# rubengooj/pl-slam

Hardware: AMD Instinct MI355X
Metric: stereo pairs/sec (1500 ORB + 200 LBD BF-match) (higher is better)
Workload: dtype fp4; 1 GPU; C2: synthetic 752x480 stereo stream, 1500 ORB + 200 LBD per image, ORB+LBD L<->R and prev<->curr, mutual + ratio (StVO::match), then StereoFrame's gates over the L<->R tables (config_kitti.yaml:25-...; mutual=True, distinct_batches_in_rotation=3, stereo_gates=True, kernel=k_scan_sym_mfma_i, mfma_form=0

## Files before the change

### plslam_amd/csrc/hamming.hip

```cpp
#include "mfma_h_common.hpp"
#include "stereo_gates_dev.hpp"

namespace plslam {

typedef const __attribute__((address_space(4))) uint32_t* sptr_t;
typedef uint32_t u32x4 __attribute__((ext_vector_type(4), aligned(4)));

__device__ __forceinline__ uint32_t bcnt0(uint32_t x)
{
    uint32_t r;
    asm("v_bcnt_u32_b32 %0, %1, 0" : "=v"(r) : "v"(x));
    return r;
}
__device__ __forceinline__ uint32_t med3_u32(uint32_t a, uint32_t b, uint32_t c)
{
    uint32_t r;
    asm("v_med3_u32 %0, %1, %2, %3" : "=v"(r) : "v"(a), "v"(b), "v"(c));
    return r;
}
__device__ __forceinline__ uint32_t make_key_s(uint32_t d, uint32_t j_uniform)
{
    uint32_t r;
    asm("v_lshl_or_b32 %0, %1, 23, %2" : "=v"(r) : "v"(d), "s"(j_uniform));
    return r;
// ... 134 lines not shown
    for (int k = 0; k < WPQ_QUERIES_PER_WAVE; ++k) {
        uint32_t k0 = b[k][0], k1 = b[k][1];
#pragma unroll
        for (int m = 32; m >= 1; m >>= 1)
            merge2(k0, k1, (uint32_t)__shfl_xor((int)k0, m), (uint32_t)__shfl_xor((int)k1, m));
        if (lane == 0 && q0 + k < nq) g_(reinterpret_cast<gvec2_t*>(sc.keys))[q0 + k] = gvec2_t{k0, k1};
    }
}

constexpr int SYM_TILE_ROW_U16 = 72;
constexpr int SYM_TILE_U16 = 64 * SYM_TILE_ROW_U16;

typedef uint16_t u16x2 __attribute__((ext_vector_type(2)));

constexpr uint32_t SYM_INVALID_BIAS = 512;
__device__ __forceinline__ uint32_t pk_keys(uint32_t w, uint32_t ipair_uniform)
{
    uint32_t r;
    asm("v_lshl_or_b32 %0, %1, 6, %2" : "=v"(r) : "v"(w), "s"(ipair_uniform));
    return r;
}
__device__ __forceinline__ uint32_t key16_to_32(uint32_t c, uint32_t i_base)
{
    return c >= 0x8000u ? KEY_NONE : (((c >> 6) << KEY_IDX_BITS) | (i_base + (c & 63u)));
}

__device__ __forceinline__ void sym_column_reduce(const uint16_t* __restrict__ col, uint32_t& b0,
                                                  uint32_t& b1)
{
    const uint4* cp = reinterpret_cast<const uint4*>(col);
    b0 = 0xFFFFFFFFu;
    b1 = 0xFFFFFFFFu;
#pragma unroll
    for (int v = 0; v < 8; ++v) {
        const uint4 w4 = cp[v];
        const uint32_t w[4] = {w4.x, w4.y, w4.z, w4.w};
#pragma unroll
        for (int u = 0; u < 4; ++u) {
            const int i_lo = 8 * v + 2 * u;
            const uint32_t key = pk_keys(w[u], (uint32_t)(((i_lo + 1) << 16) | i_lo));
            pk_push2(b0, b1, key);
        }
    }
}

__global__ void __launch_bounds__(256)
k_scan_symmetric(const SymDesc* __restrict__ syms, const BlockDesc* __restrict__ blocks,
                 int32_t* __restrict__ zero, int nzero)
{
    __shared__ __attribute__((aligned(16))) uint16_t lds[4 * SYM_TILE_U16];

    if (blockIdx.x == 0)
        for (int i = threadIdx.x; i < nzero; i += 256) g_(zero)[i] = 0;

    const int wg = xcd_remap_(blockIdx.x, gridDim.x);
    const BlockDesc bd = blocks[wg];
    if (bd.item < 0) return;
    const SymDesc sd = syms[bd.item];
    const int n1 = sd.n1, n2 = sd.n2;
    const int lane = threadIdx.x & 63;
    const int wave = __builtin_amdgcn_readfirstlane((int)(threadIdx.x >> 6));
    const int i0 = bd.row0 + 64 * wave;
    if (i0 >= n1) return;
    const int iblk = i0 >> 6;
    const int row = i0 + lane;
    const uint32_t bias = row < n1 ? 0u : SYM_INVALID_BIAS;
    const int rrow = row < n1 ? row : n1 - 1;

    uint32_t q[8];
    {
        const auto qp = g_(reinterpret_cast<const u32x4*>(sd.a + (size_t)rrow * 32));
        const u32x4 a = qp[0], b = qp[1];
        q[0] = a.x; q[1] = a.y; q[2] = a.z; q[3] = a.w;
        q[4] = b.x; q[5] = b.y; q[6] = b.z; q[7] = b.w;
    }
    uint16_t* tile = lds + wave * SYM_TILE_U16;
    uint16_t* wr = tile + lane;
    const uint16_t* col = tile + lane * SYM_TILE_ROW_U16;
    const auto part = g_(reinterpret_cast<gvec2_t*>(sd.part21)) + (size_t)iblk * n2;
    sptr_t tp = (sptr_t)(uintptr_t)sd.b;

    uint32_t rb0 = KEY_NONE, rb1 = KEY_NONE;
    for (int j0 = 0; j0 < n2; j0 += 64) {
        const int jc = n2 - j0 < 64 ? n2 - j0 : 64;
        int jj = 0;
        for (; jj + 4 <= jc; jj += 4) {
            sptr_t t = tp + (size_t)(j0 + jj) * 8;
            const uint32_t d0 = PLSLAM_DIST8B(q, t, bias);
            const uint32_t d1 = PLSLAM_DIST8B(q, t + 8, bias);
            const uint32_t d2 = PLSLAM_DIST8B(q, t + 16, bias);
            const uint32_t d3 = PLSLAM_DIST8B(q, t + 24, bias);
            wr[(jj + 0) * SYM_TILE_ROW_U16] = (uint16_t)d0;
            wr[(jj + 1) * SYM_TILE_ROW_U16] = (uint16_t)d1;
            wr[(jj + 2) * SYM_TILE_ROW_U16] = (uint16_t)d2;
            wr[(jj + 3) * SYM_TILE_ROW_U16] = (uint16_t)d3;
            best2_push(rb0, rb1, make_key_s(d0, (uint32_t)(j0 + jj)));
            best2_push(rb0, rb1, make_key_s(d1, (uint32_t)(j0 + jj + 1)));
            best2_push(rb0, rb1, make_key_s(d2, (uint32_t)(j0 + jj + 2)));
            best2_push(rb0, rb1, make_key_s(d3, (uint32_t)(j0 + jj + 3)));
        }
        for (; jj < jc; ++jj) {
            sptr_t t = tp + (size_t)(j0 + jj) * 8;
            const uint32_t d = PLSLAM_DIST8B(q, t, bias);
            wr[jj * SYM_TILE_ROW_U16] = (uint16_t)d;
            best2_push(rb0, rb1, make_key_s(d, (uint32_t)(j0 + jj)));
        }
        __builtin_amdgcn_fence(__ATOMIC_RELEASE, "wavefront");
        __builtin_amdgcn_wave_barrier();
        __builtin_amdgcn_fence(__ATOMIC_ACQUIRE, "wavefront");
        uint32_t c0p, c1p;
        sym_column_reduce(col, c0p, c1p);
        {
            const uint32_t e0 = c0p & 0xFFFFu, o0 = c0p >> 16, e1 = c1p & 0xFFFFu, o1 = c1p >> 16;
            const uint32_t m0 = umin_(e0, o0);
            const uint32_t m1 = umin_(umax_(e0, o0), umin_(e1, o1));
            if (lane < jc)
                part[j0 + lane] = gvec2_t{key16_to_32(m0, (uint32_t)i0), key16_to_32(m1, (uint32_t)i0)};
        }
        __builtin_amdgcn_fence(__ATOMIC_RELEASE, "wavefront");
        __builtin_amdgcn_wave_barrier();
        __builtin_amdgcn_fence(__ATOMIC_ACQUIRE, "wavefront");
    }
    if (row < n1) g_(reinterpret_cast<gvec2_t*>(sd.keys12))[row] = gvec2_t{rb0, rb1};
}

constexpr int SYM4_SUBTILE_U16 = 16 * SYM_TILE_ROW_U16;

__global__ void __launch_bounds__(64)
k_scan_symmetric_r4(const SymDesc* __restrict__ syms, const BlockDesc* __restrict__ blocks,
                    int32_t* __restrict__ zero, int nzero)
{
    __shared__ __attribute__((aligned(16))) uint16_t tile[4 * SYM4_SUBTILE_U16];

    if (blockIdx.x == 0)
        for (int i = threadIdx.x; i < nzero; i += 64) g_(zero)[i] = 0;

    const int wg = xcd_remap_(blockIdx.x, gridDim.x);
    const BlockDesc bd = blocks[wg];
    if (bd.item < 0) return;
    const SymDesc sd = syms[bd.item];
    const int n1 = sd.n1, n2 = sd.n2;
    const int lane = threadIdx.x;
    const int i0 = bd.row0;
    const int iblk = i0 >> 8;

    uint32_t q0[8], c1[8], c2[8], c3[8];
    uint32_t bias[4];
    {
        uint32_t qr[4][8];
#pragma unroll
        for (int r = 0; r < 4; ++r) {
            const int row = i0 + 64 * r + lane;
            bias[r] = row < n1 ? 0u : SYM_INVALID_BIAS;
            const int rrow = row < n1 ? row : n1 - 1;
            const auto qp = g_(reinterpret_cast<const u32x4*>(sd.a + (size_t)rrow * 32));
            const u32x4 a = qp[0], b = qp[1];
            qr[r][0] = a.x; qr[r][1] = a.y; qr[r][2] = a.z; qr[r][3] = a.w;
            qr[r][4] = b.x; qr[r][5] = b.y; qr[r][6] = b.z; qr[r][7] = b.w;
        }
#pragma unroll
        for (int k = 0; k < 8; ++k) {
            q0[k] = qr[0][k];
            c1[k] = qr[0][k] ^ qr[1][k];
            c2[k] = qr[0][k] ^ qr[2][k];
            c3[k] = qr[0][k] ^ qr[3][k];
        }
    }
    uint16_t* wr = tile + lane;
    const uint16_t* col = tile + (lane >> 4) * SYM4_SUBTILE_U16 + (lane & 15) * SYM_TILE_ROW_U16;
    const uint32_t col_i_base = (uint32_t)(i0 + 64 * (lane >> 4));
    const auto part = g_(reinterpret_cast<gvec2_t*>(sd.part21)) + (size_t)iblk * n2;
    sptr_t tp = (sptr_t)(uintptr_t)sd.b;

    uint32_t rb[4][2];
#pragma unroll
    for (int r = 0; r < 4; ++r) rb[r][0] = rb[r][1] = KEY_NONE;

#define PLSLAM_SYM4_ROW(T, JJ)                                                                    \
    {                                                                                             \
        uint32_t x[8];                                                                            \
        _Pragma("unroll") for (int k = 0; k < 8; ++k) x[k] = q0[k] ^ (T)[k];                      \
        const uint32_t e0 = bcnt_acc_(x[7], bcnt_acc_(x[6], bcnt_acc_(x[5], bcnt_acc_(x[4],       \
                            bcnt_acc_(x[3], bcnt_acc_(x[2], bcnt_acc_(x[1], bcnt_acc_(x[0], bias[0])))))))); \
        const uint32_t e1 = bcnt_acc_(x[7] ^ c1[7], bcnt_acc_(x[6] ^ c1[6], bcnt_acc_(x[5] ^ c1[5], \
                            bcnt_acc_(x[4] ^ c1[4], bcnt_acc_(x[3] ^ c1[3], bcnt_acc_(x[2] ^ c1[2], \
                            bcnt_acc_(x[1] ^ c1[1], bcnt_acc_(x[0] ^ c1[0], bias[1]))))))));      \
        const uint32_t e2 = bcnt_acc_(x[7] ^ c2[7], bcnt_acc_(x[6] ^ c2[6], bcnt_acc_(x[5] ^ c2[5], \
                            bcnt_acc_(x[4] ^ c2[4], bcnt_acc_(x[3] ^ c2[3], bcnt_acc_(x[2] ^ c2[2], \
                            bcnt_acc_(x[1] ^ c2[1], bcnt_acc_(x[0] ^ c2[0], bias[2]))))))));      \
        const uint32_t e3 = bcnt_acc_(x[7] ^ c3[7], bcnt_acc_(x[6] ^ c3[6], bcnt_acc_(x[5] ^ c3[5], \
                            bcnt_acc_(x[4] ^ c3[4], bcnt_acc_(x[3] ^ c3[3], bcnt_acc_(x[2] ^ c3[2], \
                            bcnt_acc_(x[1] ^ c3[1], bcnt_acc_(x[0] ^ c3[0], bias[3]))))))));      \
        wr[0 * SYM4_SUBTILE_U16 + (JJ) * SYM_TILE_ROW_U16] = (uint16_t)e0;                        \
        wr[1 * SYM4_SUBTILE_U16 + (JJ) * SYM_TILE_ROW_U16] = (uint16_t)e1;                        \
        wr[2 * SYM4_SUBTILE_U16 + (JJ) * SYM_TILE_ROW_U16] = (uint16_t)e2;                        \
        wr[3 * SYM4_SUBTILE_U16 + (JJ) * SYM_TILE_ROW_U16] = (uint16_t)e3;                        \
        const uint32_t jkey = (uint32_t)(j0 + (JJ));                                              \
        best2_push(rb[0][0], rb[0][1], make_key_s(e0, jkey));                                     \
        best2_push(rb[1][0], rb[1][1], make_key_s(e1, jkey));                                     \
        best2_push(rb[2][0], rb[2][1], make_key_s(e2, jkey));                                     \
        best2_push(rb[3][0], rb[3][1], make_key_s(e3, jkey));                                     \
    }

    for (int j0 = 0; j0 < n2; j0 += 16) {
        const int jc = n2 - j0 < 16 ? n2 - j0 : 16;
        int jj = 0;
        for (; jj + 4 <= jc; jj += 4) {
            sptr_t t = tp + (size_t)(j0 + jj) * 8;
            PLSLAM_SYM4_ROW(t, jj + 0)
            PLSLAM_SYM4_ROW(t + 8, jj + 1)
            PLSLAM_SYM4_ROW(t + 16, jj + 2)
            PLSLAM_SYM4_ROW(t + 24, jj + 3)
        }
        for (; jj < jc; ++jj) {
            sptr_t t = tp + (size_t)(j0 + jj) * 8;
            PLSLAM_SYM4_ROW(t, jj)
        }
        __builtin_amdgcn_fence(__ATOMIC_RELEASE, "wavefront");
        __builtin_amdgcn_wave_barrier();
        __builtin_amdgcn_fence(__ATOMIC_ACQUIRE, "wavefront");
        uint32_t c0p, c1p;
        sym_column_reduce(col, c0p, c1p);
        const uint32_t ev0 = c0p & 0xFFFFu, od0 = c0p >> 16, ev1 = c1p & 0xFFFFu, od1 = c1p >> 16;
        uint32_t k0 = key16_to_32(umin_(ev0, od0), col_i_base);
        uint32_t k1 = key16_to_32(umin_(umax_(ev0, od0), umin_(ev1, od1)), col_i_base);
        merge2(k0, k1, (uint32_t)__shfl_xor((int)k0, 16), (uint32_t)__shfl_xor((int)k1, 16));
        merge2(k0, k1, (uint32_t)__shfl_xor((int)k0, 32), (uint32_t)__shfl_xor((int)k1, 32));
        if (lane < jc) part[j0 + lane] = gvec2_t{k0, k1};
        __builtin_amdgcn_fence(__ATOMIC_RELEASE, "wavefront");
        __builtin_amdgcn_wave_barrier();
        __builtin_amdgcn_fence(__ATOMIC_ACQUIRE, "wavefront");
    }
#undef PLSLAM_SYM4_ROW
#pragma unroll
    for (int r = 0; r < 4; ++r) {
        const int row = i0 + 64 * r + lane;
        if (row < n1) g_(reinterpret_cast<gvec2_t*>(sd.keys12))[row] = gvec2_t{rb[r][0], rb[r][1]};
    }
}

__global__ void __launch_bounds__(256)
k_merge_partials(const SymDesc* __restrict__ syms, const BlockDesc* __restrict__ blocks)
{
    const BlockDesc bd = blocks[blockIdx.x];
    const SymDesc sd = syms[bd.item];
    const int j = bd.row0 + (int)threadIdx.x;
    if (j >= sd.n2) return;
    const auto part = g_(reinterpret_cast<const gvec2_t*>(sd.part21));
    uint32_t b0 = KEY_NONE, b1 = KEY_NONE;
    for (int ib = 0; ib < sd.n_iblk; ++ib) {
        const gvec2_t p = part[(size_t)ib * sd.n2 + j];
        merge2(b0, b1, p.x, p.y);
    }
    g_(reinterpret_cast<gvec2_t*>(sd.keys21))[j] = gvec2_t{b0, b1};
}

__device__ __forceinline__ int ratio_pick(uint32_t k0, uint32_t k1, float nnr)
{
    if (k1 == KEY_NONE) return -1;
    const float d0 = (float)(k0 >> KEY_IDX_BITS);
    const float d1n = __fmul_rn((float)(k1 >> KEY_IDX_BITS), nnr);
    return d0 < d1n ? (int)(k0 & KEY_IDX_MASK) : -1;
}

template <class FetchKb>
__device__ __forceinline__ void finalize_row(const ProblemDesc& p, const int i1, const plslam_stereo_gate_problem* __restrict__ gates,
                                             FetchKb fetch_kb, const gvec2_t* pre = nullptr)
{
    int m = -1;
    bool accepted = false, cleared = false;
    uint2 k = make_uint2(KEY_NONE, KEY_NONE);
    uint2 kb = make_uint2(KEY_NONE, KEY_NONE);
    bool check = false;
    if (i1 < p.n1) {
        if (p.nsplit > 1) {
            const auto tmp = g_(reinterpret_cast<const gvec2_t*>(p.split_tmp));
            uint32_t b0 = KEY_NONE, b1 = KEY_NONE;
            for (int s = 0; s < p.nsplit; ++s) {
                const gvec2_t q = tmp[(size_t)s * p.n1 + i1];
                const uint32_t off = (uint32_t)(s * p.cstep);
                merge2(b0, b1, q.x == KEY_NONE ? KEY_NONE : q.x + off, q.y == KEY_NONE ? KEY_NONE : q.y + off);
            }
            k = make_uint2(b0, b1);
            g_(reinterpret_cast<gvec2_t*>(p.keys12_out))[i1] = gvec2_t{k.x, k.y};
        } else if (pre) {
            k = make_uint2(pre->x, pre->y);
        } else {
            const gvec2_t kv = __builtin_nontemporal_load(g_(reinterpret_cast<const gvec2_t*>(p.keys12)) + i1);
            k = make_uint2(kv.x, kv.y);
        }
        m = ratio_pick(k.x, k.y, p.nnr);
        accepted = m >= 0;
        if (!accepted && p.keep_prior) m = g_(p.matches_12)[i1];
        if (m >= 0 && p.mutual) {
            check = m < p.n2;
            if (check) kb = fetch_kb(m);
            else { m = -1; cleared = true; }
        }
    }
    bool ok = true;
    if (!p.lazy21) {
        if (check) ok = ratio_pick(kb.x, kb.y, p.nnr) == i1;
    } else {
        const uint32_t mm = check ? (uint32_t)m : 0xFFFFFFFFu;
        uint32_t lb = 0xFFFFFFFFu;
#define PLSLAM_FIN_ROT(S)                                                                           \
        {                                                                                          \
            const uint32_t px = (uint32_t)__builtin_amdgcn_update_dpp(-1, (int)k.x, 0x120 + (S), 0xf, 0xf, false); \
            const uint32_t py = (uint32_t)__builtin_amdgcn_update_dpp(-1, (int)k.y, 0x120 + (S), 0xf, 0xf, false); \
            const uint32_t b = (px != KEY_NONE && (px & KEY_IDX_MASK) == mm) ? (px >> KEY_IDX_BITS)  \
                                                                           : (py == KEY_NONE ? 0xFFFFFFFFu : (py >> KEY_IDX_BITS)); \
            lb = lb < b ? lb : b;                                                                  \
        }
        PLSLAM_FIN_ROT(1) PLSLAM_FIN_ROT(2) PLSLAM_FIN_ROT(3) PLSLAM_FIN_ROT(4) PLSLAM_FIN_ROT(5)
        PLSLAM_FIN_ROT(6) PLSLAM_FIN_ROT(7) PLSLAM_FIN_ROT(8) PLSLAM_FIN_ROT(9) PLSLAM_FIN_ROT(10)
        PLSLAM_FIN_ROT(11) PLSLAM_FIN_ROT(12) PLSLAM_FIN_ROT(13) PLSLAM_FIN_ROT(14) PLSLAM_FIN_ROT(15)
#undef PLSLAM_FIN_ROT
        if (check) {
            ok = kb.x != KEY_NONE && (int)(kb.x & KEY_IDX_MASK) == i1;
            if (ok) {
                const float d0 = (float)(kb.x >> KEY_IDX_BITS);
                const uint32_t hi = kb.y == KEY_NONE ? 0xFFFFFFFFu : (kb.y >> KEY_IDX_BITS);
                const uint32_t lo = hi < lb ? hi : lb;
                if (hi != 0xFFFFFFFFu && !(d0 < __fmul_rn((float)hi, p.nnr))) {
                    ok = false;
                } else if (lo != 0xFFFFFFFFu && d0 < __fmul_rn((float)lo, p.nnr)) {
                    ok = true;
                } else {
                    uint32_t second = kb.y;
                    const auto b = g_(reinterpret_cast<const u32x4*>(p.d2 + (size_t)m * 32));
                    const u32x4 b_lo = b[0], b_hi = b[1];
                    const int base = i1 & ~15;
                    for (int q = 0; q < 16; ++q) {
                        const int i = base + q;
                        const bool use = i != i1 && i < p.n1;
                        const auto a = g_(reinterpret_cast<const u32x4*>(p.d1 + (size_t)(use ? i : i1) * 32));
                        const u32x4 a_lo = a[0], a_hi = a[1];
                        const uint32_t d = __popc(a_lo.x ^ b_lo.x) + __popc(a_lo.y ^ b_lo.y) + __popc(a_lo.z ^ b_lo.z) +
                                           __popc(a_lo.w ^ b_lo.w) + __popc(a_hi.x ^ b_hi.x) + __popc(a_hi.y ^ b_hi.y) +
                                           __popc(a_hi.z ^ b_hi.z) + __popc(a_hi.w ^ b_hi.w);
                        const uint32_t cand = use ? ((d << KEY_IDX_BITS) | (uint32_t)i) : KEY_NONE;
                        second = second < cand ? second : cand;
                    }
                    ok = ratio_pick(kb.x, second, p.nnr) == i1;
                }
            }
        }
    }
    if (check && !ok) { m = -1; cleared = true; }
    if (i1 < p.n1) {
        __builtin_nontemporal_store(m, g_(p.matches_12) + i1);
        if (p.matches_16) g_(p.matches_16)[i1] = (int16_t)m;
    }
    if (p.n_matches) {
        const int delta = (int)__popcll(__ballot(accepted)) - (int)__popcll(__ballot(cleared));
        if ((threadIdx.x & 63) == 0 && delta) (void)atomic_add_global(p.n_matches, delta);
    }
    if (gates && p.gate >= 0) {
        const plslam_stereo_gate_problem q = gates[p.gate];
        const int kept = i1 < p.n1 ? stereo_gate_row(q, i1, m) : 0;
        const unsigned long long bal = __ballot(kept);
        if (q.n_stereo && (threadIdx.x & 63) == 0 && bal) (void)atomic_add_global(q.n_stereo, (int)__popcll(bal));
    }
}

__global__ void __launch_bounds__(256)
k_finalize(const ProblemDesc* __restrict__ probs, const BlockDesc* __restrict__ blocks,
           const plslam_stereo_gate_problem* __restrict__ gates, int nblocks, int per_xcd)
{
  const int nslots = per_xcd > 0 ? 8 * per_xcd : nblocks;
  for (int b = blockIdx.x; b < nslots; b += gridDim.x) {
    const int blk = per_xcd > 0 ? (b & 7) * per_xcd + (b >> 3) : b;
    if (blk >= nblocks) continue;
    const BlockDesc bd = blocks[blk];
    if (bd.item < 0) continue;
    const ProblemDesc p = probs[bd.item];
    finalize_row(p, bd.row0 + (int)threadIdx.x, gates, [&](int m) {
        const gvec2_t kv = g_(reinterpret_cast<const gvec2_t*>(p.keys21))[m];
        return make_uint2(kv.x, kv.y);
    });
  }
}

template <int NT>
__global__ void __launch_bounds__(NT)
k_post_fused(const ProblemDesc* __restrict__ probs, const plslam_stereo_gate_problem* __restrict__ gates, int nprob)
{
    extern __shared__ __attribute__((aligned(16))) uint2 kb_lds[];
    for (int pi = blockIdx.x; pi < nprob; pi += gridDim.x) {
        const ProblemDesc p = probs[pi];
        const MhLayout L(p.n2);
        const int nwb = (p.n1 + 255) >> 8, n2p = L.slots_padded(), nslots = 32 * L.ntiles;
        const auto part = g_(p.part21);
        if (pi != (int)blockIdx.x) __syncthreads();
        const auto k12 = g_(reinterpret_cast<const gvec2_t*>(p.keys12));
        gvec2_t kcur = gvec2_t{KEY_NONE, KEY_NONE};
        if ((int)threadIdx.x < p.n1) kcur = __builtin_nontemporal_load(k12 + threadIdx.x);
        constexpr int PF = NT >= 1024 ? 2 : 4;
        for (int s0_ = (int)threadIdx.x; s0_ < nslots; s0_ += NT * PF) {
            uint32_t b0[PF], b1[PF], sx[PF];
            int j[PF];
#pragma unroll
            for (int q = 0; q < PF; ++q) {
                const int slot = s0_ + NT * q;
                j[q] = slot < nslots ? L.row_of(slot >> 5, slot & 31) : p.n2;
                b0[q] = b1[q] = KEY_NONE;
                sx[q] = 0xFFFFFFFFu;
            }
            for (int wb = 0; wb < nwb; ++wb) {
                uint32_t e[PF];
#pragma unroll
                for (int q = 0; q < PF; ++q) e[q] = j[q] < p.n2 ? __builtin_nontemporal_load(&part[(size_t)wb * n2p + s0_ + NT * q]) : 0xFFFFFFFFu;
#pragma unroll
                for (int q = 0; q < PF; ++q) {
                    const uint32_t e0 = e[q] >> 9, e1 = ((e[q] & 511u) << 8) | 255u;
                    const uint32_t k = ((e0 >> 8) << KEY_IDX_BITS) | ((e0 & 255u) + 256u * (uint32_t)wb);
                    sx[q] = k < b0[q] ? e1 : sx[q];
                    b1[q] = umin_(b1[q], umax_(b0[q], k));
                    b0[q] = umin_(b0[q], k);
                }
            }
#pragma unroll
            for (int q = 0; q < PF; ++q) {
                if (j[q] >= p.n2) continue;
                if (b0[q] < (257u << KEY_IDX_BITS)) {
                    b1[q] = umin_(b1[q], ((sx[q] >> 8) << KEY_IDX_BITS) | KEY_IDX_MASK);
                    if (b1[q] >= (257u << KEY_IDX_BITS)) b1[q] = KEY_NONE;
                } else {
                    b0[q] = b1[q] = KEY_NONE;
                }
                kb_lds[j[q]] = make_uint2(b0[q], b1[q]);
            }
        }
        __syncthreads();
#pragma unroll 1
        for (int r0 = 0; r0 < p.n1; r0 += NT) {
            const int inext = r0 + NT + (int)threadIdx.x;
            gvec2_t knext = gvec2_t{KEY_NONE, KEY_NONE};
            if (inext < p.n1) knext = __builtin_nontemporal_load(k12 + inext);
            finalize_row(p, r0 + (int)threadIdx.x, gates, [&](int m) { return kb_lds[m]; }, &kcur);
            kcur = knext;
        }
    }
}

__global__ void __launch_bounds__(256)
k_scatter_counts(const int32_t* __restrict__ src, int32_t* const* __restrict__ dst, int32_t n)
{
    const int i = blockIdx.x * 256 + threadIdx.x;
    if (i < n && g_(dst)[i]) *g_(g_(dst)[i]) = g_(src)[i];
}

__global__ void __launch_bounds__(256)
k_unpack_keys(const uint32_t* __restrict__ keys, int32_t n, int32_t* __restrict__ idx,
              int32_t* __restrict__ dist)
{
    const int i = blockIdx.x * 256 + threadIdx.x;
    if (i >= n) return;
    const uint32_t k = g_(keys)[i];
    idx[i] = k == KEY_NONE ? -1 : (int32_t)(k & KEY_IDX_MASK);
    dist[i] = k == KEY_NONE ? INT32_MAX : (int32_t)(k >> KEY_IDX_BITS);
}

int scan_rows_per_block(int variant, int block_threads)
{
    return variant == PLSLAM_SCAN_WAVE_PER_QUERY ? WPQ_QUERIES_PER_BLOCK : block_threads;
}

int launch_scan(const plslam_ctx* ctx, int variant, int block_threads, const ScanDesc* d_scans,
                const BlockDesc* d_blocks, int nblocks, int32_t* d_zero, int nzero, hipStream_t s)
{
    (void)ctx;
    if (nblocks <= 0) {
        if (nzero > 0) PLSLAM_HIP_CHECK(hipMemsetAsync(d_zero, 0, sizeof(int32_t) * nzero, s));
        return PLSLAM_OK;
    }
    if (variant == PLSLAM_SCAN_WAVE_PER_QUERY) {
        hipLaunchKernelGGL(k_scan_wave_per_query, dim3(nblocks), dim3(256), 0, s, d_scans, d_blocks, d_zero,
                           nzero);
        PLSLAM_HIP_CHECK(hipGetLastError());
        return PLSLAM_OK;
    }
    PLSLAM_REQUIRE(variant == PLSLAM_SCAN_LANE_PER_QUERY, PLSLAM_EINVAL);
    switch (block_threads) {
        case 256:
            hipLaunchKernelGGL(k_scan_lane_per_query<256>, dim3(nblocks), dim3(256), 0, s, d_scans,
                               d_blocks, d_zero, nzero);
            break;
        case 512:
            hipLaunchKernelGGL(k_scan_lane_per_query<512>, dim3(nblocks), dim3(512), 0, s, d_scans,
                               d_blocks, d_zero, nzero);
            break;
        case 1024:
            hipLaunchKernelGGL(k_scan_lane_per_query<1024>, dim3(nblocks), dim3(1024), 0, s, d_scans,
                               d_blocks, d_zero, nzero);
            break;
        default:
            PLSLAM_REQUIRE(!"scan_block must be 256, 512 or 1024", PLSLAM_EINVAL);
    }
    PLSLAM_HIP_CHECK(hipGetLastError());
    return PLSLAM_OK;
}

int sym_rows_per_block(int rows_per_lane) { return 256; (void)rows_per_lane; }
int sym_rows_per_partial(int rows_per_lane) { return rows_per_lane == 4 ? 256 : 64; }

int launch_scan_sym(int rows_per_lane, const SymDesc* d_sym, const BlockDesc* d_blocks, int nblocks,
                    int32_t* d_zero, int nzero, hipStream_t s)
{
    if (nblocks <= 0) return PLSLAM_OK;
    if (rows_per_lane == 4)
        hipLaunchKernelGGL(k_scan_symmetric_r4, dim3(nblocks), dim3(64), 0, s, d_sym, d_blocks, d_zero, nzero);
    else
        hipLaunchKernelGGL(k_scan_symmetric, dim3(nblocks), dim3(256), 0, s, d_sym, d_blocks, d_zero, nzero);
    PLSLAM_HIP_CHECK(hipGetLastError());
    return PLSLAM_OK;
}

int launch_merge_partials(const SymDesc* d_sym, const BlockDesc* d_blocks, int nblocks, hipStream_t s)
{
    if (nblocks <= 0) return PLSLAM_OK;
    hipLaunchKernelGGL(k_merge_partials, dim3(nblocks), dim3(256), 0, s, d_sym, d_blocks);
    PLSLAM_HIP_CHECK(hipGetLastError());
    return PLSLAM_OK;
}

constexpr int POST_FUSED_THREADS = 256;
int launch_post_fused(const ProblemDesc* d_probs, int nprob, const plslam_stereo_gate_problem* d_gates, size_t lds_bytes,
                      hipStream_t s)
{
    if (nprob <= 0) return PLSLAM_OK;
    hipLaunchKernelGGL(k_post_fused<POST_FUSED_THREADS>, dim3(nprob), dim3(POST_FUSED_THREADS), lds_bytes, s, d_probs, d_gates, nprob);
    PLSLAM_HIP_CHECK(hipGetLastError());
    return PLSLAM_OK;
}

int launch_finalize(const ProblemDesc* d_probs, const BlockDesc* d_blocks, int nblocks,
                    const plslam_stereo_gate_problem* d_gates, hipStream_t s, int grid_cap, bool xcd_chunks, int dealt_row)
{
    if (nblocks <= 0) return PLSLAM_OK;
    const int per_xcd = dealt_row > 0 ? dealt_row : (xcd_chunks && nblocks >= 64 ? (nblocks + 7) / 8 : 0);
    const int nslots = per_xcd > 0 ? 8 * per_xcd : nblocks;
    int grid = grid_cap > 0 && grid_cap < nslots ? grid_cap : nslots;
    if (per_xcd > 0 && grid < nslots) grid = grid >= 8 ? grid & ~7 : 8;
    hipLaunchKernelGGL(k_finalize, dim3(grid), dim3(256), 0, s, d_probs, d_blocks, d_gates, nblocks, per_xcd);
    PLSLAM_HIP_CHECK(hipGetLastError());
    return PLSLAM_OK;
}

int launch_scatter_counts(const int32_t* d_src, int32_t* const* d_dst, int32_t n, hipStream_t s)
{
    if (n <= 0) return PLSLAM_OK;
    hipLaunchKernelGGL(k_scatter_counts, dim3((n + 255) / 256), dim3(256), 0, s, d_src, d_dst, n);
    PLSLAM_HIP_CHECK(hipGetLastError());
    return PLSLAM_OK;
}

int launch_unpack_keys(const uint32_t* d_keys, int32_t n, int32_t* d_idx, int32_t* d_dist,
                       hipStream_t s)
{
    if (n <= 0) return PLSLAM_OK;
    hipLaunchKernelGGL(k_unpack_keys, dim3((n + 255) / 256), dim3(256), 0, s, d_keys, n, d_idx,
                       d_dist);
    PLSLAM_HIP_CHECK(hipGetLastError());
    return PLSLAM_OK;
}

}
```

### plslam_amd/csrc/hamming_mfma_h.hip

```cpp
#include "mfma_h_common.hpp"

#include <type_traits>

namespace plslam {


int mh_slot_of_column(int n2, int j) { return MhLayout(n2).slot_of(j); }
__host__ __device__ inline int mh_block_row(int w, int mt, int m) { return 128 * mt + 32 * w + 16 * ((m >> 2) & 1) + (m & 3) + 4 * (m >> 3); }

#if PLSLAM_BUILD_LEGACY_SCANS
template <bool DIRECTED>
__global__ void __launch_bounds__(256, 3)
k_scan_sym_mfma_h(const SymDesc* __restrict__ syms, const BlockDesc* __restrict__ blocks, int32_t* __restrict__ zero, int nzero)
{
    constexpr int ROWX_STRIDE = 33;
    constexpr int PARK_OFF = 2 * MH_TILE_BYTES;
    constexpr int SMEM_BYTES = PARK_OFF + 4 * 16 * 64 * 8;
    static_assert(SMEM_BYTES >= 4 * 64 * ROWX_STRIDE * 4, "the transpose must fit");
    __shared__ __attribute__((aligned(16))) uint8_t smem[SMEM_BYTES];
    __shared__ __attribute__((aligned(16))) uint32_t colstage[MH_CGROUP * 256];
    __shared__ __attribute__((aligned(16))) uint32_t rawring[3][256];
    uint8_t* const btile = smem;
    u32x2_t* const park = reinterpret_cast<u32x2_t*>(smem + PARK_OFF) + (threadIdx.x >> 6) * (16 * 64) + (threadIdx.x & 63);

// ... 51 lines not shown
    const int ej = tid >> 3, ewd4 = (tid & 7) * 4;
    const PLSLAM_GLOBAL char* const bbytes = (const PLSLAM_GLOBAL char*) sd.b;
    auto load_raw = [&](int t) __attribute__((always_inline)) -> uint32_t {
        const int tc = t < ntiles ? t : ntiles - 1;
        const int gbase = (tc >> 4) * MH_GROUP_ROWS;
        const uint32_t s = tc < nfull ? (uint32_t)MH_GROUP : (uint32_t)rag_s;
        uint32_t row = __umul24((uint32_t)ej, s) + (uint32_t)(tc & 15);
        const uint32_t last = (uint32_t)(n2 - 1 - gbase);
        row = row < last ? row : last;
        return *reinterpret_cast<gcu32_t>(bbytes + (size_t)gbase * 32 + (row * 32u + (uint32_t)ewd4));
    };
    auto load_raw_async = [&](int t, int slot) __attribute__((always_inline)) {
        const int tc = t < ntiles ? t : ntiles - 1;
        const int gbase = (tc >> 4) * MH_GROUP_ROWS;
        const uint32_t s = tc < nfull ? (uint32_t)MH_GROUP : (uint32_t)rag_s;
        uint32_t row = __umul24((uint32_t)ej, s) + (uint32_t)(tc & 15);
        const uint32_t last = (uint32_t)(n2 - 1 - gbase);
        row = row < last ? row : last;
        const uint32_t voff = row * 32u + (uint32_t)ewd4;
        const PLSLAM_GLOBAL char* sbase = bbytes + (size_t)gbase * 32;
        const uint32_t lds_dst = (uint32_t)(uintptr_t)(&rawring[slot][64 * w]);
        uint32_t keep;
        asm volatile("s_mov_b32 %0, m0\n\ts_mov_b32 m0, %3\n\ts_nop 0\n\tglobal_load_lds_dword %1, %2\n\ts_mov_b32 m0, %0"
                     : "=&s"(keep) : "v"(voff), "s"(sbase), "s"(lds_dst) : "memory");
    };
    auto take_raw = [&](int slot) __attribute__((always_inline)) -> uint32_t {
        asm volatile("s_waitcnt vmcnt(2)" ::: "memory");
        return rawring[slot][tid];
    };
    auto expand_store = [&](uint32_t raw, int buf, int tn) __attribute__((always_inline)) {
        uint8_t* dst = btile + buf * MH_TILE_BYTES + ej * MH_ROW_STRIDE + ewd4 * 4;
        i32x4 v = expand_dword_fp4<false>(raw);
        if (tn >= nfull) {
            const int vm = (int)(__umul24((uint32_t)rag_s, (uint32_t)ej) + (uint32_t)(tn & 15)) < rest ? -1 : 0;
            v &= i32x4{vm, vm, vm, vm};
        }
        *reinterpret_cast<i32x4*>(dst) = v;
    };

    int wt0 = 0, wt1 = ntiles < MH_WINDOW ? ntiles : MH_WINDOW;
    int ring_slot = 1;

    const uint64_t part_u = (uint64_t)(uintptr_t)part;
    const uint64_t part_s = ((uint64_t)(uint32_t)__builtin_amdgcn_readfirstlane((int)(part_u >> 32)) << 32) |
                            (uint32_t)__builtin_amdgcn_readfirstlane((int)(uint32_t)part_u);
    auto combine_columns = [&](int kb) __attribute__((always_inline)) {
        if (DIRECTED) return;
        uint32_t l_;
        asm volatile("v_mbcnt_lo_u32_b32 %0, -1, 0\n\tv_mbcnt_hi_u32_b32 %0, -1, %0" : "=&v"(l_));
        const uint32_t* const src = colstage + 512 * w + (((l_ & 32u) << 3) | (l_ & 31u));
        uint32_t p[8];
#pragma unroll
        for (int v = 0; v < 4; ++v) { p[2 * v] = src[64 * v]; p[2 * v + 1] = src[64 * v + 32]; }
        uint32_t lo[4], hi[4];
#pragma unroll
        for (int q = 0; q < 4; ++q) { lo[q] = pk_min16(p[2 * q], p[2 * q + 1]); hi[q] = pk_max16(p[2 * q], p[2 * q + 1]); }
        auto pk_merge = [](uint32_t& a0, uint32_t& a1, uint32_t c0, uint32_t c1) {
            const uint32_t m = pk_max16(a0, c0);
            a0 = pk_min16(a0, c0);
            a1 = pk_min16(m, pk_min16(a1, c1));
        };
        pk_merge(lo[0], hi[0], lo[1], hi[1]);
        pk_merge(lo[2], hi[2], lo[3], hi[3]);
        pk_merge(lo[0], hi[0], lo[2], hi[2]);
        const uint32_t e0 = lo[0] & 0xFFFFu, e1 = hi[0] & 0xFFFFu, u0 = lo[0] >> 16, u1 = hi[0] >> 16;
        uint32_t k0 = e0 + (e0 & 0xFF80u), k1 = e1 + (e1 & 0xFF80u);
        merge2(k0, k1, u0 + (u0 & 0xFF80u) + 128u, u1 + (u1 & 0xFF80u) + 128u);
        const uint32_t slot4 = (uint32_t)(256 * kb + 64 * w) * 4u;
        if (!wide_part) {
            const uint32_t e = (k0 << 9) | (k1 >> 8);
            PLSLAM_GLOBAL uint32_t* dst = (PLSLAM_GLOBAL uint32_t*)((PLSLAM_GLOBAL char*)(uintptr_t)(part_s + slot4) + 4u * l_);
            __builtin_nontemporal_store(e, dst);
        } else {
            const u32x2_t e = {k0, k1};
            PLSLAM_GLOBAL u32x2_t* dst = (PLSLAM_GLOBAL u32x2_t*)((PLSLAM_GLOBAL char*)(uintptr_t)(part_s + 2u * slot4) + 8u * l_);
            __builtin_nontemporal_store(e, dst);
        }
    };
    auto push_groups = [&](int t) __attribute__((always_inline)) {
        const uint32_t gtag = (uint32_t)(((((t - wt0) >> 4) ^ w) & 3) << 5) * 0x00010001u;
#pragma unroll
        for (int r = 0; r < 16; ++r) {
            const u32x2_t v = park[r * 64];
            uint32_t b0 = v.x, b1 = v.y;
            pk_push2(b0, b1, gm[r] ^ gtag);
            park[r * 64] = u32x2_t{b0, b1};
            gm[r] = 0xFFFFFFFFu;
        }
    };
    auto finish_columns = [&](int t, uint32_t cm) __attribute__((always_inline)) {
        if (DIRECTED) { asm volatile("" ::"v"(cm)); return; }
        cstage[(t & (MH_CGROUP - 1)) * 256 + lane] = cm;
    };

#define PLSLAM_MH_EPI_ROW(R)                                                                       \
    {                                                                                              \
        uint32_t kcv = kc[R];                                                                      \
        gm[R] = pk_min16(gm[R], kcv);                                                              \
        if (!DIRECTED) {                                                                           \
            if (MASKED) kcv |= ((R) < PLSLAM_MH_NV_LO ? 0u : 0x0000FFFFu) | ((R) < PLSLAM_MH_NV_LO - 128 ? 0u : 0xFFFF0000u); \
            if ((R) & 1) cm1 = pk_min16(cm1, kcv); else cm = pk_min16(cm, kcv);                    \
        }                                                                                          \
    }
    uint32_t kc[16];
    auto tile_step = [&](int t, auto u_tag, bool with_prev, auto masked_tag) __attribute__((always_inline)) {
        constexpr bool MASKED = decltype(masked_tag)::value;
        constexpr int U = decltype(u_tag)::value;
        __syncthreads();
        const uint8_t* bt = btile + (U & 1) * MH_TILE_BYTES + c * MH_ROW_STRIDE + 16 * g;
        uint32_t cm = 0xFFFFFFFFu, cm1 = 0xFFFFFFFFu;
        auto read_b = [&](int ks) __attribute__((always_inline)) -> i32x4 {
            (void)t;
            return *reinterpret_cast<const i32x4*>(bt + 32 * ks);
        };
        i32x4 bfr[MH_KSTEPS];
        bfr[0] = read_b(0);
        bfr[1] = read_b(1);
        const uint32_t raw_next = take_raw(ring_slot);
        if (t >= nfull && ((t & 15) == 0 || (t & 15) == lim_part)) {
            const uint32_t pen = lane_lim() == (t & 15) ? COL_PENALTY : 0u;
#pragma unroll
            for (int r = 0; r < 16; ++r) seed[r] += pen;
            asm volatile("" : "+v"(seed));
        }
        const f32x16 cseed = __builtin_bit_cast(f32x16, seed);
        f32x16 m0, m1;
#define PLSLAM_MH_MMA(ACC, MT, KS, CIN)                                                            \
        {                                                                                          \
            const i32x8 a8 = {afrag[MT][KS].x, afrag[MT][KS].y, afrag[MT][KS].z, afrag[MT][KS].w, 0, 0, 0, 0}; \
            const i32x8 b8 = {bfr[KS].x, bfr[KS].y, bfr[KS].z, bfr[KS].w, 0, 0, 0, 0};             \
            ACC = __builtin_amdgcn_mfma_scale_f32_32x32x64_f8f6f4(a8, b8, CIN, 4, 4, 0, scale_a, 0, scale_b); \
            asm volatile("" : "+v"(ACC));                  \
            __builtin_amdgcn_sched_barrier(0);                                                     \
        }
#define PLSLAM_MH_EPI2(R)                                                                          \
        {                                                                                          \
            { PLSLAM_MH_EPI_ROW(R) PLSLAM_MH_EPI_ROW((R) + 1) }                                    \
            __builtin_amdgcn_sched_barrier(0);                                                     \
        }
        __builtin_amdgcn_sched_barrier(0);
        PLSLAM_MH_EPI2(0)  PLSLAM_MH_MMA(m0, 0, 0, cseed)
        PLSLAM_MH_EPI2(2)  PLSLAM_MH_MMA(m1, 1, 0, cseed)
        bfr[2] = read_b(2);
        PLSLAM_MH_EPI2(4)  PLSLAM_MH_MMA(m0, 0, 1, m0)
        PLSLAM_MH_EPI2(6)  PLSLAM_MH_MMA(m1, 1, 1, m1)
        bfr[3] = read_b(3);
        PLSLAM_MH_EPI2(8)  PLSLAM_MH_MMA(m0, 0, 2, m0)
        PLSLAM_MH_EPI2(10) PLSLAM_MH_MMA(m1, 1, 2, m1)
        PLSLAM_MH_EPI2(12) PLSLAM_MH_MMA(m0, 0, 3, m0)
        PLSLAM_MH_EPI2(14) PLSLAM_MH_MMA(m1, 1, 3, m1)
#undef PLSLAM_MH_EPI2
#undef PLSLAM_MH_MMA
        expand_store(raw_next, (U + 1) & 1, t + 1);
        load_raw_async(t + 4, ring_slot);
        ring_slot = ring_slot == 2 ? 0 : ring_slot + 1;
        if (with_prev) {
            if (!DIRECTED && U == 1 && ((t - 1) & (MH_CGROUP - 1)) == 0 && t - 9 >= wt0) {
                combine_columns((t - 9) >> 3);
                __syncthreads();
            }
            finish_columns(t - 1, pk_min16(cm, cm1));
            if (U == 0 && ((t - 1) & (MH_GROUP - 1)) == MH_GROUP - 1) push_groups(t - 1);
        }
#pragma unroll
        for (int r = 0; r < 16; ++r) {
            const float f0 = m0[r], f1 = m1[r];
            kc[r] = pack_acc(f0, f1);
        }
    };
    auto epilogue = [&](int t, auto masked_tag) __attribute__((always_inline)) {
        constexpr bool MASKED = decltype(masked_tag)::value;
        uint32_t cm = 0xFFFFFFFFu, cm1 = 0xFFFFFFFFu;
        PLSLAM_MH_EPI_ROW(0) PLSLAM_MH_EPI_ROW(1) PLSLAM_MH_EPI_ROW(2) PLSLAM_MH_EPI_ROW(3)
        PLSLAM_MH_EPI_ROW(4) PLSLAM_MH_EPI_ROW(5) PLSLAM_MH_EPI_ROW(6) PLSLAM_MH_EPI_ROW(7)
        PLSLAM_MH_EPI_ROW(8) PLSLAM_MH_EPI_ROW(9) PLSLAM_MH_EPI_ROW(10) PLSLAM_MH_EPI_ROW(11)
        PLSLAM_MH_EPI_ROW(12) PLSLAM_MH_EPI_ROW(13) PLSLAM_MH_EPI_ROW(14) PLSLAM_MH_EPI_ROW(15)
        finish_columns(t, pk_min16(cm, cm1));
    };
    auto pipeline = [&](auto masked_tag) __attribute__((always_inline)) {
#pragma unroll
        for (int r = 0; r < 16; ++r) kc[r] = 0xFFFFFFFFu;
        for (int tb = wt0; tb < wt1; tb += 4) {
            tile_step(tb, std::integral_constant<int, 0>{}, tb != wt0, masked_tag);
            if (tb + 1 < wt1) tile_step(tb + 1, std::integral_constant<int, 1>{}, true, masked_tag);
            if (tb + 2 < wt1) tile_step(tb + 2, std::integral_constant<int, 2>{}, true, masked_tag);
            if (tb + 3 < wt1) tile_step(tb + 3, std::integral_constant<int, 3>{}, true, masked_tag);
        }
        if (!DIRECTED && ((wt1 - 1) & (MH_CGROUP - 1)) == 0 && wt1 - 9 >= wt0) {
            __syncthreads();
            combine_columns((wt1 - 9) >> 3);
            __syncthreads();
        }
        epilogue(wt1 - 1, masked_tag);
        push_groups(wt1 - 1);
    };
#undef PLSLAM_MH_EPI_ROW

    auto finish_rows = [&]() __attribute__((always_inline)) {
        uint32_t* rowx = reinterpret_cast<uint32_t*>(smem) + w * (64 * ROWX_STRIDE);
        u32x2_t rb[16];
#pragma unroll
        for (int r = 0; r < 16; ++r) rb[r] = park[r * 64];
        __syncthreads();
#pragma unroll
        for (int r = 0; r < 16; ++r) {
            const int lrow = 16 * g + r;
            rowx[lrow * ROWX_STRIDE + c] = __builtin_amdgcn_perm(rb[r].y, rb[r].x, 0x05040100u);
            rowx[(32 + lrow) * ROWX_STRIDE + c] = __builtin_amdgcn_perm(rb[r].y, rb[r].x, 0x07060302u);
        }
        __builtin_amdgcn_fence(__ATOMIC_RELEASE, "wavefront");
        __builtin_amdgcn_wave_barrier();
        __builtin_amdgcn_fence(__ATOMIC_ACQUIRE, "wavefront");
        uint32_t k0 = 0xFFFFFFFFu, k1 = 0xFFFFFFFFu;
        const uint32_t* mine = rowx + lane * ROWX_STRIDE;
#pragma unroll 8
        for (int cls = 0; cls < 32; ++cls) {
            const uint32_t e = mine[cls];
            merge2(k0, k1, (e << 16) | (uint32_t)cls, (e & 0xFFFF0000u) | (uint32_t)cls);
        }
        const int row = iw + lane + (lane & 32) * 3;
        if (row < n1) {
            const gu2_t out = (gu2_t) reinterpret_cast<u32x2_t*>(sd.keys12) + row;
            const gcu32x4_t ap = (gcu32x4_t)(araw + (size_t)row * 8);
            const u32x4_t a_lo = ap[0], a_hi = ap[1];
            auto group_of = [&](uint32_t k, uint32_t& jbase, uint32_t& cnt) {
                const uint32_t t0 = (uint32_t)wt0 + (((k >> 21) & 3u) << 4);
                const uint32_t s = t0 < (uint32_t)nfull ? (uint32_t)MH_GROUP : (uint32_t)rag_s;
                jbase = (t0 >> 4) * MH_GROUP_ROWS + s * (k & 0xFFFFu);
                cnt = s;
            };
            auto rescan = [&](uint32_t jbase, uint32_t cnt, uint32_t& best, uint32_t& second) {
                best = second = KEY_NONE;
                const uint32_t left = (uint32_t)n2 - jbase;
                const uint32_t nvalid = cnt < left ? cnt : left;
                const PLSLAM_GLOBAL char* const rb = bbytes + (size_t)jbase * 32;
#pragma unroll
                for (int k0_ = 0; k0_ < MH_GROUP; k0_ += 4) {
                    u32x4_t bl[4], bh[4];
#pragma unroll
                    for (int q = 0; q < 4; ++q) {
                        const uint32_t kk = (uint32_t)(k0_ + q) < nvalid ? (uint32_t)(k0_ + q) : nvalid - 1u;
                        const gcu32x4_t bp = (gcu32x4_t)(rb + kk * 32u);
                        bl[q] = bp[0];
                        bh[q] = bp[1];
                    }
#pragma unroll
                    for (int q = 0; q < 4; ++q) {
                        const uint32_t d = hamming256(a_lo, a_hi, bl[q], bh[q]);
                        const uint32_t cand = (uint32_t)(k0_ + q) < nvalid ? ((d << KEY_IDX_BITS) | (jbase + (uint32_t)(k0_ + q))) : KEY_NONE;
                        second = umin_(second, umax_(best, cand));
                        best = umin_(best, cand);
                    }
                }
            };
            uint32_t r0 = KEY_NONE, r1 = KEY_NONE;
            if ((k0 >> 16) <= KEY16_MAX) {
                uint32_t jb, cnt, in2;
                group_of(k0, jb, cnt);
                rescan(jb, cnt, r0, in2);
                if ((k1 >> 16) <= KEY16_MAX) {
                    uint32_t jb1, cnt1;
                    group_of(k1, jb1, cnt1);
                    uint32_t o1 = ((k1 >> 23) << KEY_IDX_BITS) | jb1;
                    if ((sd.flags & 1) && (o1 >> KEY_IDX_BITS) <= (in2 >> KEY_IDX_BITS)) {
                        uint32_t b1, s1;
                        rescan(jb1, cnt1, b1, s1);
                        o1 = b1;
                    }
                    r1 = umin_(in2, o1);
                } else {
                    r1 = in2;
                }
            }
            if (wt0 > 0) {
                const u32x2_t prev = *out;
                merge2(r0, r1, prev.x, prev.y);
            }
            *out = u32x2_t{r0, r1};
        }
        __builtin_amdgcn_fence(__ATOMIC_RELEASE, "wavefront");
        __builtin_amdgcn_wave_barrier();
    };

    for (;;) {
#pragma unroll
        for (int r = 0; r < 16; ++r) park[r * 64] = u32x2_t{0xFFFFFFFFu, 0xFFFFFFFFu};
        expand_store(load_raw(wt0), 0, wt0);
        load_raw_async(wt0 + 1, 1);
        load_raw_async(wt0 + 2, 2);
        load_raw_async(wt0 + 3, 0);
        ring_slot = 1;
        if (!rows_ragged) pipeline(std::false_type{}); else pipeline(std::true_type{});
        __syncthreads();
        combine_columns((wt1 - 1) >> 3);
        finish_rows();
        if (wt1 == ntiles) break;
        __syncthreads();
        wt0 = wt1;
        wt1 = ntiles < wt0 + MH_WINDOW ? ntiles : wt0 + MH_WINDOW;
    }
}
#endif

template <int PARTS, bool FIX>
__global__ void __launch_bounds__(256)
k_merge_fix16(const SymDesc* __restrict__ syms, const BlockDesc* __restrict__ blocks, int nblocks)
{
  for (int blk = blockIdx.x; blk < nblocks; blk += gridDim.x) {
    constexpr int COLS = 256 / PARTS;
    constexpr int SPT = PARTS == 1 ? MH_MERGE_SPT : 1;
    __shared__ uint32_t red[PARTS > 1 ? 512 : 2];
    const BlockDesc bd = blocks[blk];
    const SymDesc sd = syms[bd.item];
    const int jl = (int)threadIdx.x % COLS, part_id = (int)threadIdx.x / COLS;
    const MhLayout L(sd.n2);
    const gcu32_t part = (gcu32_t) sd.part21;
    const int nwb = (sd.n1 + 255) >> 8;
    const int n2p = (MH_TILE_N * L.ntiles + 255) & ~255;
    int slot[SPT], j[SPT];
    uint32_t b0[SPT], b1[SPT], s0[SPT];
#pragma unroll
    for (int q = 0; q < SPT; ++q) {
        slot[q] = bd.row0 + jl + 256 * q;
        j[q] = slot[q] < MH_TILE_N * L.ntiles ? L.row_of(slot[q] >> 5, slot[q] & 31) : sd.n2;
        if (j[q] >= sd.n2) slot[q] = 0;
        b0[q] = b1[q] = KEY_NONE;
        s0[q] = 0xFFFFFFFFu;
    }
    auto wide = [](uint32_t k17, uint32_t wb) -> uint32_t {
        return ((k17 >> 8) << KEY_IDX_BITS) | ((k17 & 255u) + 256u * wb);
    };
    if (PARTS == 1 && !FIX) {
        constexpr int WB = MH_MERGE_WB;
        for (int wb0 = 0; wb0 < nwb; wb0 += WB) {
            uint32_t e[WB][SPT];
#pragma unroll
            for (int u = 0; u < WB; ++u) {
                if (wb0 + u < nwb) {
#pragma unroll
                    for (int q = 0; q < SPT; ++q)
                        e[u][q] = __builtin_nontemporal_load(&part[(size_t)(wb0 + u) * n2p + slot[q]]);
                }
            }
#pragma unroll
            for (int u = 0; u < WB; ++u) {
                if (wb0 + u < nwb) {
#pragma unroll
                    for (int q = 0; q < SPT; ++q) {
                        const uint32_t k = wide(e[u][q] >> 9, (uint32_t)(wb0 + u)), e1 = ((e[u][q] & 511u) << 8) | 255u;
                        s0[q] = k < b0[q] ? e1 : s0[q];
                        b1[q] = umin_(b1[q], umax_(b0[q], k));
                        b0[q] = umin_(b0[q], k);
                    }
                }
            }
        }
    } else
#pragma unroll 2
    for (int wb = part_id; wb < nwb; wb += PARTS) {
        uint32_t e0[SPT], e1[SPT];
#pragma unroll
        for (int q = 0; q < SPT; ++q) {
            if (FIX) {
                const gu2c_t pp = (gu2c_t) part + ((size_t)wb * n2p + slot[q]);
                const u32x2_t e = __builtin_nontemporal_load(pp);
                e0[q] = e.x; e1[q] = e.y;
            } else {
                const uint32_t e = __builtin_nontemporal_load(&part[(size_t)wb * n2p + slot[q]]);
                e0[q] = e >> 9; e1[q] = ((e & 511u) << 8) | 255u;
            }
        }
#pragma unroll
        for (int q = 0; q < SPT; ++q) {
            const uint32_t k = wide(e0[q], (uint32_t)wb);
            s0[q] = k < b0[q] ? e1[q] : s0[q];
            b1[q] = umin_(b1[q], umax_(b0[q], k));
            b0[q] = umin_(b0[q], k);
        }
    }
#pragma unroll
    for (int q = 0; q < SPT; ++q) {
        if (j[q] < sd.n2 && b0[q] < (257u << KEY_IDX_BITS)) {
            const uint32_t k1 = FIX ? wide(s0[q], (b0[q] & KEY_IDX_MASK) >> 8) : (((s0[q] >> 8) << KEY_IDX_BITS) | KEY_IDX_MASK);
            b1[q] = umin_(b1[q], k1);
            if (b1[q] >= (257u << KEY_IDX_BITS)) b1[q] = KEY_NONE;
        } else {
            b0[q] = b1[q] = KEY_NONE;
        }
    }
    if (PARTS > 1) {
        if (blk != (int)blockIdx.x) __syncthreads();
        red[2 * threadIdx.x] = b0[0];
        red[2 * threadIdx.x + 1] = b1[0];
        __syncthreads();
        if (part_id == 0) {
#pragma unroll
            for (int q = 1; q < PARTS; ++q) merge2(b0[0], b1[0], red[2 * (q * COLS + jl)], red[2 * (q * COLS + jl) + 1]);
        }
    }
#pragma unroll
    for (int q = 0; q < SPT; ++q) {
        if (part_id == 0 && j[q] < sd.n2) {
            if (FIX && b0[q] != KEY_NONE) {
                const gcu32_t araw = (gcu32_t) reinterpret_cast<const uint32_t*>(sd.a);
                const gcu32x4_t bp = (gcu32x4_t)((gcu32_t) reinterpret_cast<const uint32_t*>(sd.b) + (size_t)j[q] * 8);
                const u32x4_t b_lo = bp[0], b_hi = bp[1];
                const uint32_t i0 = b0[q] & KEY_IDX_MASK, ibase = i0 & ~15u;
#pragma unroll
                for (int k = 0; k < 16; ++k) {
                    const uint32_t i = ibase + (uint32_t)k;
                    const bool ok = i != i0 && i < (uint32_t)sd.n1;
                    const gcu32x4_t ap = (gcu32x4_t)(araw + (size_t)(ok ? i : i0) * 8);
                    const u32x4_t a_lo = ap[0], a_hi = ap[1];
                    const uint32_t d = hamming256(a_lo, a_hi, b_lo, b_hi);
                    b1[q] = umin_(b1[q], ok ? ((d << KEY_IDX_BITS) | i) : KEY_NONE);
                }
            }
            ((gu2_t) reinterpret_cast<u32x2_t*>(sd.keys21))[j[q]] = u32x2_t{b0[q], b1[q]};
        }
    }
  }
}

int merge_fix16_cols(int parts) { return parts >= 16 ? 16 : parts >= 4 ? 64 : 256 * MH_MERGE_SPT; }

int launch_merge_fix16(const SymDesc* d_sym, const BlockDesc* d_blocks, int nblocks, int parts, bool fix, hipStream_t s, int grid_cap)
{
    if (nblocks <= 0) return PLSLAM_OK;
    const int grid = grid_cap > 0 && grid_cap < nblocks ? grid_cap : nblocks;
#define PLSLAM_MH_MERGE(P) { if (fix) hipLaunchKernelGGL((k_merge_fix16<P, true>), dim3(grid), dim3(256), 0, s, d_sym, d_blocks, nblocks); \
                             else hipLaunchKernelGGL((k_merge_fix16<P, false>), dim3(grid), dim3(256), 0, s, d_sym, d_blocks, nblocks); }
    if (parts >= 16) PLSLAM_MH_MERGE(16)
    else if (parts >= 4) PLSLAM_MH_MERGE(4)
    else PLSLAM_MH_MERGE(1)
#undef PLSLAM_MH_MERGE
    PLSLAM_HIP_CHECK(hipGetLastError());
    return PLSLAM_OK;
}

#if PLSLAM_BUILD_LEGACY_SCANS
int launch_scan_sym_mfma_h(const SymDesc* d_sym, const BlockDesc* d_blocks, int nblocks, int32_t* d_zero, int nzero,
                           bool directed, hipStream_t s)
{
    if (nblocks <= 0) return PLSLAM_OK;
    if (directed) hipLaunchKernelGGL((k_scan_sym_mfma_h<true>), dim3(nblocks), dim3(256), 0, s, d_sym, d_blocks, d_zero, nzero);
    else hipLaunchKernelGGL((k_scan_sym_mfma_h<false>), dim3(nblocks), dim3(256), 0, s, d_sym, d_blocks, d_zero, nzero);
    PLSLAM_HIP_CHECK(hipGetLastError());
    return PLSLAM_OK;
}
#endif

}
```

Before: 1.713 million stereo pairs/s.

## Skip DPP lower-bound scan when undecided and pack merge keys for med3 top-2

In the lazy mutual-check finalize, the 15-step DPP rotation that computes a lower bound now runs only when some lane in the wave still needs it after the cheap ratio test. The rotation also tracks plain second-distance minima instead of per-lane conditional selects. In the merge kernel, each partial entry is packed with its block index into a single sortable word, so the top-2 update becomes a med3 plus a min. The original fields are unpacked once at the end. The packed path is limited to at most 64 row blocks, and the bit-packing must stay exactly equivalent to the old key and second-distance encoding.

```diff
diff --git a/plslam_amd/csrc/hamming.hip b/plslam_amd/csrc/hamming.hip
--- a/plslam_amd/csrc/hamming.hip
+++ b/plslam_amd/csrc/hamming.hip
@@ -460,49 +460,46 @@
     if (!p.lazy21) {
         if (check) ok = ratio_pick(kb.x, kb.y, p.nnr) == i1;
     } else {
-        const uint32_t mm = check ? (uint32_t)m : 0xFFFFFFFFu;
-        uint32_t lb = 0xFFFFFFFFu;
-#define PLSLAM_FIN_ROT(S)                                                                           \
-        {                                                                                          \
-            const uint32_t px = (uint32_t)__builtin_amdgcn_update_dpp(-1, (int)k.x, 0x120 + (S), 0xf, 0xf, false); \
-            const uint32_t py = (uint32_t)__builtin_amdgcn_update_dpp(-1, (int)k.y, 0x120 + (S), 0xf, 0xf, false); \
-            const uint32_t b = (px != KEY_NONE && (px & KEY_IDX_MASK) == mm) ? (px >> KEY_IDX_BITS)  \
-                                                                           : (py == KEY_NONE ? 0xFFFFFFFFu : (py >> KEY_IDX_BITS)); \
-            lb = lb < b ? lb : b;                                                                  \
-        }
-        PLSLAM_FIN_ROT(1) PLSLAM_FIN_ROT(2) PLSLAM_FIN_ROT(3) PLSLAM_FIN_ROT(4) PLSLAM_FIN_ROT(5)
-        PLSLAM_FIN_ROT(6) PLSLAM_FIN_ROT(7) PLSLAM_FIN_ROT(8) PLSLAM_FIN_ROT(9) PLSLAM_FIN_ROT(10)
-        PLSLAM_FIN_ROT(11) PLSLAM_FIN_ROT(12) PLSLAM_FIN_ROT(13) PLSLAM_FIN_ROT(14) PLSLAM_FIN_ROT(15)
+        const float d0 = (float)(kb.x >> KEY_IDX_BITS);
+        const uint32_t hi = kb.y == KEY_NONE ? 0xFFFFFFFFu : (kb.y >> KEY_IDX_BITS);
+        if (check) ok = kb.x != KEY_NONE && (int)(kb.x & KEY_IDX_MASK) == i1 &&
+                        !(hi != 0xFFFFFFFFu && !(d0 < __fmul_rn((float)hi, p.nnr)));
+        const bool need_lb = check && ok;
+        bool undecided = false;
+        if (__ballot(need_lb)) {
+            const uint32_t mm = check ? (uint32_t)m : 0xFFFFFFFFu;
+            const uint32_t sd = k.y == KEY_NONE ? 0xFFFFFFFFu : (k.y >> KEY_IDX_BITS);
+            const uint32_t bi = k.x == KEY_NONE ? 0xFFFFFFFEu : (k.x & KEY_IDX_MASK);
+            uint32_t S = 0xFFFFFFFFu, nd = 0xFFFFFFFFu;
+#define PLSLAM_FIN_ROT(R)                                                                           \
+            {                                                                                      \
+                S = umin_(S, (uint32_t)__builtin_amdgcn_update_dpp(0, (int)sd, 0x120 + (R), 0xf, 0xf, true)); \
+                nd = umin_(nd, (uint32_t)__builtin_amdgcn_update_dpp(0, (int)bi, 0x120 + (R), 0xf, 0xf, true) ^ mm); \
+            }
+            PLSLAM_FIN_ROT(1) PLSLAM_FIN_ROT(2) PLSLAM_FIN_ROT(3) PLSLAM_FIN_ROT(4) PLSLAM_FIN_ROT(5)
+            PLSLAM_FIN_ROT(6) PLSLAM_FIN_ROT(7) PLSLAM_FIN_ROT(8) PLSLAM_FIN_ROT(9) PLSLAM_FIN_ROT(10)
+            PLSLAM_FIN_ROT(11) PLSLAM_FIN_ROT(12) PLSLAM_FIN_ROT(13) PLSLAM_FIN_ROT(14) PLSLAM_FIN_ROT(15)
 #undef PLSLAM_FIN_ROT
-        if (check) {
-            ok = kb.x != KEY_NONE && (int)(kb.x & KEY_IDX_MASK) == i1;
-            if (ok) {
-                const float d0 = (float)(kb.x >> KEY_IDX_BITS);
-                const uint32_t hi = kb.y == KEY_NONE ? 0xFFFFFFFFu : (kb.y >> KEY_IDX_BITS);
-                const uint32_t lo = hi < lb ? hi : lb;
-                if (hi != 0xFFFFFFFFu && !(d0 < __fmul_rn((float)hi, p.nnr))) {
-                    ok = false;
-                } else if (lo != 0xFFFFFFFFu && d0 < __fmul_rn((float)lo, p.nnr)) {
-                    ok = true;
-                } else {
-                    uint32_t second = kb.y;
-                    const auto b = g_(reinterpret_cast<const u32x4*>(p.d2 + (size_t)m * 32));
-                    const u32x4 b_lo = b[0], b_hi = b[1];
-                    const int base = i1 & ~15;
-                    for (int q = 0; q < 16; ++q) {
-                        const int i = base + q;
-                        const bool use = i != i1 && i < p.n1;
-                        const auto a = g_(reinterpret_cast<const u32x4*>(p.d1 + (size_t)(use ? i : i1) * 32));
-                        const u32x4 a_lo = a[0], a_hi = a[1];
-                        const uint32_t d = __popc(a_lo.x ^ b_lo.x) + __popc(a_lo.y ^ b_lo.y) + __popc(a_lo.z ^ b_lo.z) +
-                                           __popc(a_lo.w ^ b_lo.w) + __popc(a_hi.x ^ b_hi.x) + __popc(a_hi.y ^ b_hi.y) +
-                                           __popc(a_hi.z ^ b_hi.z) + __popc(a_hi.w ^ b_hi.w);
-                        const uint32_t cand = use ? ((d << KEY_IDX_BITS) | (uint32_t)i) : KEY_NONE;
-                        second = second < cand ? second : cand;
-                    }
-                    ok = ratio_pick(kb.x, second, p.nnr) == i1;
-                }
+            const uint32_t lo = nd == 0 ? 0xFFFFFFFFu : (hi < S ? hi : S);
+            undecided = need_lb & !((lo != 0xFFFFFFFFu) & (d0 < __fmul_rn((float)lo, p.nnr)));
+        }
+        if (undecided) {
+            uint32_t second = kb.y;
+            const auto b = g_(reinterpret_cast<const u32x4*>(p.d2 + (size_t)m * 32));
+            const u32x4 b_lo = b[0], b_hi = b[1];
+            const int base = i1 & ~15;
+            for (int q = 0; q < 16; ++q) {
+                const int i = base + q;
+                const bool use = i != i1 && i < p.n1;
+                const auto a = g_(reinterpret_cast<const u32x4*>(p.d1 + (size_t)(use ? i : i1) * 32));
+                const u32x4 a_lo = a[0], a_hi = a[1];
+                const uint32_t d = __popc(a_lo.x ^ b_lo.x) + __popc(a_lo.y ^ b_lo.y) + __popc(a_lo.z ^ b_lo.z) +
+                                   __popc(a_lo.w ^ b_lo.w) + __popc(a_hi.x ^ b_hi.x) + __popc(a_hi.y ^ b_hi.y) +
+                                   __popc(a_hi.z ^ b_hi.z) + __popc(a_hi.w ^ b_hi.w);
+                const uint32_t cand = use ? ((d << KEY_IDX_BITS) | (uint32_t)i) : KEY_NONE;
+                second = second < cand ? second : cand;
             }
+            ok = second != KEY_NONE && d0 < __fmul_rn((float)(second >> KEY_IDX_BITS), p.nnr);
         }
     }
     if (check && !ok) { m = -1; cleared = true; }
diff --git a/plslam_amd/csrc/hamming_mfma_h.hip b/plslam_amd/csrc/hamming_mfma_h.hip
--- a/plslam_amd/csrc/hamming_mfma_h.hip
+++ b/plslam_amd/csrc/hamming_mfma_h.hip
@@ -377,6 +377,19 @@
 }
 #endif
 
+__device__ __forceinline__ uint32_t med3_u32_(uint32_t a, uint32_t b, uint32_t c)
+{
+    uint32_t r;
+    asm("v_med3_u32 %0, %1, %2, %3" : "=v"(r) : "v"(a), "v"(b), "v"(c));
+    return r;
+}
+__device__ __forceinline__ uint32_t pack_part(uint32_t e, uint32_t block_uniform)
+{
+    uint32_t r;
+    asm("v_mad_u32_u24 %0, %1, %2, %3\n\tv_add_u32 %0, %4, %0" : "=&v"(r) : "v"(e >> 17), "s"(0x7E0000u), "v"(e), "s"(block_uniform << 17));
+    return r;
+}
+
 template <int PARTS, bool FIX>
 __global__ void __launch_bounds__(256)
 k_merge_fix16(const SymDesc* __restrict__ syms, const BlockDesc* __restrict__ blocks, int nblocks)
@@ -405,16 +418,19 @@
     auto wide = [](uint32_t k17, uint32_t wb) -> uint32_t {
         return ((k17 >> 8) << KEY_IDX_BITS) | ((k17 & 255u) + 256u * wb);
     };
-    if (PARTS == 1 && !FIX) {
+    if (PARTS == 1 && !FIX && nwb <= 64) {
         constexpr int WB = MH_MERGE_WB;
+        uint32_t c0[SPT], c1[SPT];
+#pragma unroll
+        for (int q = 0; q < SPT; ++q) c0[q] = c1[q] = 0xFFFFFFFFu;
         for (int wb0 = 0; wb0 < nwb; wb0 += WB) {
             uint32_t e[WB][SPT];
 #pragma unroll
             for (int u = 0; u < WB; ++u) {
                 if (wb0 + u < nwb) {
-#pragma unroll
-                    for (int q = 0; q < SPT; ++q)
-                        e[u][q] = __builtin_nontemporal_load(&part[(size_t)(wb0 + u) * n2p + slot[q]]);
+                    const PLSLAM_GLOBAL char* const prow = (const PLSLAM_GLOBAL char*)(part + (size_t)(wb0 + u) * n2p);
+#pragma unroll
+                    for (int q = 0; q < SPT; ++q) e[u][q] = __builtin_nontemporal_load((gcu32_t)(prow + 4u * (uint32_t)slot[q]));
                 }
             }
 #pragma unroll
@@ -422,13 +438,18 @@
                 if (wb0 + u < nwb) {
 #pragma unroll
                     for (int q = 0; q < SPT; ++q) {
-                        const uint32_t k = wide(e[u][q] >> 9, (uint32_t)(wb0 + u)), e1 = ((e[u][q] & 511u) << 8) | 255u;
-                        s0[q] = k < b0[q] ? e1 : s0[q];
-                        b1[q] = umin_(b1[q], umax_(b0[q], k));
-                        b0[q] = umin_(b0[q], k);
+                        const uint32_t c = pack_part(e[u][q], (uint32_t)(wb0 + u));
+                        c1[q] = med3_u32_(c0[q], c1[q], c);
+                        c0[q] = umin_(c0[q], c);
                     }
                 }
             }
+        }
+#pragma unroll
+        for (int q = 0; q < SPT; ++q) {
+            b0[q] = (c0[q] & 0xFF800000u) | ((c0[q] >> 9) & 0x3FFFu);
+            b1[q] = (c1[q] & 0xFF800000u) | ((c1[q] >> 9) & 0x3FFFu);
+            s0[q] = c0[q] << 8;
         }
     } else
 #pragma unroll 2
```

Result: slower. 1.693 million stereo pairs/s (-1.2%).
